# qasimyu/simuscop

Measured on AMD Instinct MI355X. Metric: simulated paired reads/sec (whole node) at 30x WGS PE150, higher is better.
Workload: dtype u32

## Files before the change

simuscop_amd/csrc/sg_emit_fast.hip:

```cpp
#include "sg_emit.h"

namespace sg {

__device__ __forceinline__ uint32_t pack4(uint32_t w) {
  return (w | (w >> 6) | (w >> 12) | (w >> 18)) & 0xFFu;
}

typedef uint32_t u32x2 __attribute__((ext_vector_type(2)));
typedef uint32_t u32x4 __attribute__((ext_vector_type(4)));

#define FAST_CTX 192u

#define BITOP_OR_AND 0xF8
#define BITOP_XOR_AND 0x78
#define BITOP_ANDN_OR 0xBA

__device__ __noinline__ uint32_t tail_word(uint32_t slot, uint32_t c, uint32_t h, uint32_t c3b, uint32_t k0, uint32_t k1) {
  uint32_t y[4];
  philox_base(slot, 2u * c + (h >> 2), 1u, c3b, k0, k1, y);
  const uint32_t l = h & 3u;
  return l == 0u ? y[0] : l == 1u ? y[1] : l == 2u ? y[2] : y[3];
}

template <int H>
__device__ __forceinline__ void sample1(uint32_t col_sh, uint32_t col_mask, uint32_t cw, uint32_t wh, uint32_t so_h, uint32_t qo_h, uint32_t cd4_w,
                                        uint32_t& acc, uint32_t& sy) {
  typedef const __attribute__((address_space(3))) uint32_t* lds_word;
  const uint32_t kv4 = (cw >> (2 * H + 4)) & 0xFCu;
  const uint32_t keepm1 = *(lds_word)(uintptr_t)(so_h + kv4);
  const uint32_t d_s = keepm1 - (wh >> 16);
  const uint32_t col16 = (wh >> col_sh) & col_mask;
  const uint32_t qa = qo_h + ((cd4_w >> (8 * (H & 3))) & 0xFFu);
  const uint32_t e = *(lds_word)(uintptr_t)(qa + col16 + FAST_CTX * 4u);
  const uint32_t d_q = (wh & 0xFFFFu) - (e & 0xFFFFu);
  const uint32_t z = __builtin_amdgcn_bitop3_b32(d_q - 1u, d_q, d_s, BITOP_ANDN_OR);
  acc = __builtin_amdgcn_bitop3_b32(acc, z, 1u << (17 + H), BITOP_OR_AND);
  sy = __builtin_amdgcn_bitop3_b32(e >> 8, e, d_q, BITOP_XOR_AND);
}

__device__ __forceinline__ void sample8(const uint32_t* code4, uint32_t lgW, uint32_t cw, const uint32_t (&x)[8],
                                        const uint32_t (&so)[8], uint32_t qo0, uint32_t qo1, uint32_t (&sw)[2], uint32_t (&qw)[2],
                                        uint32_t& acc_out) {
  const uint32_t cd4[2] = {code4[(cw >> 10) & 0xFFu], code4[(cw >> 18) & 0xFFu]};
  const uint32_t col_sh = 12u - lgW, col_mask = ((1u << lgW) - 1u) << 4;
  uint32_t acc = 0, sy[8];
  sample1<0>(col_sh, col_mask, cw, x[0], so[0], qo0, cd4[0], acc, sy[0]);
  sample1<1>(col_sh, col_mask, cw, x[1], so[1], qo1, cd4[0], acc, sy[1]);
  sample1<2>(col_sh, col_mask, cw, x[2], so[2], so[2], cd4[0], acc, sy[2]);
  sample1<3>(col_sh, col_mask, cw, x[3], so[3], so[3], cd4[0], acc, sy[3]);
  sample1<4>(col_sh, col_mask, cw, x[4], so[4], so[4], cd4[1], acc, sy[4]);
  sample1<5>(col_sh, col_mask, cw, x[5], so[5], so[5], cd4[1], acc, sy[5]);
  sample1<6>(col_sh, col_mask, cw, x[6], so[6], so[6], cd4[1], acc, sy[6]);
  sample1<7>(col_sh, col_mask, cw, x[7], so[7], so[7], cd4[1], acc, sy[7]);
#pragma unroll
  for (int g = 0; g < 2; g++) {
    const uint32_t p01 = __builtin_amdgcn_perm(sy[4 * g + 1], sy[4 * g], 0x0C0C0602u);
    const uint32_t p23 = __builtin_amdgcn_perm(sy[4 * g + 3], sy[4 * g + 2], 0x06020C0Cu);
    qw[g] = p01 | p23;
    sw[g] = __builtin_amdgcn_perm(0u, 0x47544341u, cd4[g] >> 2);
  }
  acc_out = acc;
}

__device__ __forceinline__ void store_var(uint8_t* q, uint64_t lo, uint64_t hi, uint32_t n) {
  if (n >= 8u) {
    __builtin_memcpy(q, &lo, 8);
    if (n > 8u) {
      const uint32_t k = 8u * (n - 8u);
      const uint64_t v = (lo >> k) | (hi << (64u - k));
      __builtin_memcpy(q + n - 8u, &v, 8);
    }
  } else if (n >= 4u) {
    const uint32_t a = (uint32_t)lo, b = (uint32_t)(lo >> (8u * (n - 4u)));
    __builtin_memcpy(q, &a, 4);
    if (n > 4u) __builtin_memcpy(q + n - 4u, &b, 4);
  } else if (n >= 2u) {
    const uint16_t a = (uint16_t)lo, b = (uint16_t)(lo >> (8u * (n - 2u)));
    __builtin_memcpy(q, &a, 2);
    if (n > 2u) __builtin_memcpy(q + n - 2u, &b, 2);
  } else if (n == 1u) {
    *q = (uint8_t)lo;
  }
}

constexpr uint32_t FAST_G = 63u;

template <bool PAIRED, bool DIAG>
struct FastBlock {
  const DevProfile& P;
  const DevBatch& B;
  uint32_t m, tm;
  uint32_t dg;
  uint32_t bins, TI, inv_TI, clean_cap;
  uint32_t img_at;
  const uint32_t* lut;
  const uint32_t* code4;
  bool tail_whole;
  uint32_t TIp;
  uint32_t TI16, inv_TI16;

  __device__ __forceinline__ FastBlock(const DevProfile& P_, const DevBatch& B_, uint32_t m_, uint32_t TI_, uint32_t inv_TI_,
                                       uint32_t clean_cap_, uint32_t img_at_, const uint32_t* lut_, const uint32_t* code4_)
      : P(P_), B(B_), m(m_), tm(PAIRED ? m_ : 0u), dg(DIAG ? B_.diag : 0u), bins((uint32_t)P_.bins), TI(TI_), inv_TI(inv_TI_),
        clean_cap(clean_cap_), img_at(img_at_), lut(lut_), code4(code4_) {
    tail_whole = ((uint32_t)P.L & 7u) == 7u && ((uint32_t)P.L + 7u) / 8u == TI;
    TIp = tail_whole ? TI : TI - 1u;
    TI16 = (tail_whole ? TIp - 1u : TIp) >> 1;
    inv_TI16 = TI16 ? (1u << 20) / TI16 + 1u : 0u;
  }
  __device__ __forceinline__ bool rc(bool row_bit) const { return PAIRED ? m == 1u : row_bit; }
  __device__ __forceinline__ uint2 fetch_window(bool row_bit, uint32_t idx) const {
    uint2 v;
    fetch_window(row_bit, idx, v);
    return v;
  }
  __device__ __forceinline__ void fetch_window(bool row_bit, uint32_t idx, uint2& into) const {
    __builtin_memcpy(&into, (rc(row_bit) ? B.chains2_rc : B.chains2_fwd) + (idx >> 2), 8);
  }
  __device__ __forceinline__ uint32_t c3b() const { return dev_ctx(KIND_BASE, m, B.batch_id); }
};

__device__ __forceinline__ uint64_t window_codes(uint2 w, uint32_t idx) { return (((uint64_t)w.y << 32) | w.x) >> (2u * (idx & 3u)); }

struct FastWave {
  uint32_t lane;
  FastRows rows;
  uint32_t* slow_list;
  uint2* fix_list;
  uint8_t* perm;
  uint8_t* permp;
  uint16_t* ovf;
  uint16_t* clean;
  uint32_t g;
  uint8_t* gout;
  __amdgpu_buffer_rsrc_t out_rsrc;
  uint32_t nslow, nfix;
  __device__ __forceinline__ unsigned long long lanes_below() const { return (1ull << lane) - 1ull; }
};

template <bool PAIRED, bool DIAG>
__device__ __forceinline__ void heads8(const FastBlock<PAIRED, DIAG>& k, uint32_t slot, uint32_t c, uint32_t (&x)[8]) {
  const uint32_t c3b = k.c3b();
  if (k.dg & 8u) {
#pragma unroll
    for (int z = 0; z < 8; z++) x[z] = (slot * 2654435761u) ^ (c * 40503u + z * 0x9E3779B9u);
  } else {
    philox_base(slot, 2u * c, 0, c3b, k.B.k0, k.B.k1, x);
    philox_base(slot, 2u * c + 1u, 0, c3b, k.B.k0, k.B.k1, x + 4);
  }
}

template <class S, class Fetch, class Run>
__device__ __forceinline__ void pipelined_steps(S cur, uint32_t first, uint32_t last, Fetch fetch, Run run) {
  for (uint32_t step = first; step < last; step++) {
    const S nxt = fetch(min(step + 1u, last - 1u));
    run(cur);
    cur = nxt;
  }
}

template <bool PAIRED, bool DIAG>
__device__ __forceinline__ void flush_slow(const FastBlock<PAIRED, DIAG>& k, FastWave& w) {
  const DevBatch& B = k.B;
  const uint32_t m = k.m, lane = w.lane;
  wave_lds_sync();
  uint32_t base = 0;
  if (lane == 0u) base = atomicAdd(B.slowq_count + m, w.nslow);
  base = (uint32_t)__builtin_amdgcn_readfirstlane((int)base);
  for (uint32_t b0 = 0; b0 < w.nslow; b0 += 64u) {
    const uint32_t i = b0 + lane;
    if (i < w.nslow && base + i < B.slowq_cap) {
      const uint32_t e = w.slow_list[i];
      B.slowq[(size_t)m * B.slowq_cap + base + i] = make_uint2(w.g * FAST_G + (e & 0xFFu), e >> 8);
    }
  }
  if (lane == 0u && base + w.nslow > B.slowq_cap) atomicOr((unsigned long long*)(B.totals + 3), 2ull);
  w.nslow = 0;
  wave_lds_sync();
}

template <bool PAIRED, bool DIAG>
__device__ __forceinline__ void flush_fix(const FastBlock<PAIRED, DIAG>& k, FastWave& w) {
  const DevProfile& P = k.P;
  const DevBatch& B = k.B;
  const uint32_t bins = k.bins, lane = w.lane;
  wave_lds_sync();
  __builtin_amdgcn_s_waitcnt(0x0F70);
  const uint32_t lgW = P.lgW, u_mask = (1u << (16u - lgW)) - 1u;
  const uint4* gsub = P.fast_sub + (size_t)k.tm * bins * FAST_CTX;
  const uint32_t c3b = k.c3b();
  for (uint32_t b0 = 0; b0 < w.nfix; b0 += 64u) {
    const uint2 fe = w.fix_list[b0 + lane < w.nfix ? b0 + lane : 0u];
    uint32_t todo = b0 + lane < w.nfix ? (fe.x >> 6) & 0xFFu : 0u;
    const uint32_t r = fe.x & 63u, c = fe.x >> 17, cw = fe.y;
    const uint32_t slot = w.g * FAST_G + r + B.slot_offset;
    const FastRow rr = w.rows.load(r);
    const uint32_t np = rr.np(), hl = rr.hdr_len();
    const bool whole = 8u * c + 8u <= np + (uint32_t)((np & 7u) == 7u);
    const uint32_t inv = row::inv_of(max(np, 1u));
    while (__ballot(todo != 0u) != 0ull) {
      const bool on = todo != 0u;
      const uint32_t h = on ? (uint32_t)__builtin_ctz(todo) : 0u;
      todo &= todo - 1u;
      const uint32_t i = 8u * c + h;
      const uint32_t bin = __umulhi(__umul24(i, bins), inv);
      uint32_t xw[4];
      philox_base(slot, 2u * c + (h >> 2), 0, c3b, B.k0, B.k1, xw);
      const uint32_t l = h & 3u;
      const uint32_t wh = l == 0u ? xw[0] : l == 1u ? xw[1] : l == 2u ? xw[2] : xw[3];
      const uint32_t region = c == 0u ? (h == 0u ? 128u : h == 1u ? 64u : 0u) : 0u;
      const uint32_t cdn = (cw >> (2u * h + 10u)) & 3u;
      const uint4 row = gsub[(size_t)bin * FAST_CTX + region + ((cw >> (2u * h + 6u)) & 63u)];
      const uint32_t sh = wh >> 16, h0 = row.x >> 16, h1 = row.y >> 16, h2 = row.z >> 16;
      const uint32_t jj = (uint32_t)(sh > h0) + (uint32_t)(sh > h1) + (uint32_t)(sh > h2);
      const bool amb_s = on && jj != (uint32_t)(sh >= h0) + (uint32_t)(sh >= h1) + (uint32_t)(sh >= h2);
      uint32_t kn = 0;
      uint2 e2 = make_uint2(0, 0);
      const uint32_t col = (wh & 0xFFFFu) >> (16u - lgW), uh = wh & u_mask;
      auto column = [&](uint32_t j_) {
        const uint32_t jm = max(j_, row.w & 3u);
        kn = (row.w >> (2u * jm + 2u)) & 3u;
        e2 = P.fast_alias[((((size_t)cdn * 4u + kn) * bins + bin) << lgW) + col];
      };
      if (!amb_s) column(jj);
      const bool need_tail = amb_s || (on && uh == (e2.x >> 16) && (e2.y & 0xFFu) != (e2.y >> 8));
      uint32_t wt = 0;
      if (__ballot(need_tail) != 0ull) {
        if (need_tail) wt = tail_word(slot, c, h, c3b, B.k0, B.k1);
      }
      if (__ballot(amb_s) != 0ull) {
        if (amb_s) {
          const uint32_t xs = (wh & 0xFFFF0000u) | (wt >> 16);
          column((uint32_t)(xs > row.x) + (uint32_t)(xs > row.y) + (uint32_t)(xs > row.z));
        }
      }
      const uint32_t th = e2.x >> 16;
      const bool lo_side = uh != th ? uh < th : ((uh << 16) | (wt & 0xFFFFu)) < e2.x;
      const uint32_t sym = (lo_side ? (e2.y & 0xFFu) : (e2.y >> 8)) + (uint32_t)P.min_qual;
      const uint32_t ch = (0x47544341u >> (8u * kn)) & 0xFFu;
      if (on) {
        if (whole) {
          uint8_t* rec = w.gout + rr.out_off() + hl + i;
          rec[0] = (uint8_t)ch;
          rec[np + 3u] = (uint8_t)sym;
        } else if (!rr.parked_slow()) {
          w.rows.patch_parked(r, h, ch, sym);
        }
      }
    }
  }
  w.nfix = 0;
  wave_lds_sync();
}

template <bool PAIRED, bool DIAG>
__device__ __forceinline__ void push_fix(const FastBlock<PAIRED, DIAG>& k, FastWave& w, uint32_t r, uint32_t c, uint32_t fix, uint32_t cw) {
  const unsigned long long fm = __ballot(fix != 0u);
  if (fm) {
    if (w.nfix + 64u > FIX_CAP) flush_fix(k, w);
    if (fix != 0u) w.fix_list[w.nfix + (uint32_t)__popcll(fm & w.lanes_below())] = make_uint2(r | (fix << 6) | (c << 17), cw);
    w.nfix += (uint32_t)__popcll(fm);
  }
}

__device__ __forceinline__ void stage_tables(const DevProfile& P, uint32_t tm, uint32_t TI, uint32_t* img, uint32_t img_at,
                                             uint32_t* lut, uint32_t* code4) {
  const uint32_t tid = threadIdx.x, bins = (uint32_t)P.bins, img_words = bins * P.fast_stride;
  const uint4* src = (const uint4*)(P.fast_lds + (size_t)tm * P.fast_mate_words);
  for (uint32_t i = tid; i < (img_words + 3u) / 4u; i += EMIT_THREADS) ((uint4*)img)[i] = src[i];
  const uint32_t blk_bytes = P.fast_stride * 4u;
  for (uint32_t i = tid; i < TI * LUT_ROW; i += EMIT_THREADS) {
    const uint32_t c = i / LUT_ROW, f = i - c * LUT_ROW;
    const uint32_t h = f < 8u ? f : f - 8u;
    const uint32_t pos = 8u * c + h;
    const uint32_t bin = min(pos * bins / (uint32_t)P.L, bins - 1u);
    uint32_t v = bin * blk_bytes;
    if (f < 8u && c == 0u) v += f == 0u ? 128u * 4u : f == 1u ? 64u * 4u : 0u;
    lut[i] = f < 10u ? v + img_at : 0u;
  }
  for (uint32_t i = tid; i < 256u; i += EMIT_THREADS) {
    uint32_t v = 0;
    for (uint32_t z = 0; z < 4u; z++) v |= (((i >> (2u * z)) & 3u) * 4u) << (8u * z);
    code4[i] = v;
  }
}

template <bool PAIRED>
__device__ __forceinline__ void store_name(const DevBatch& B, uint32_t m, const ReadRow& my, size_t idx, uint8_t* rec) {
  const uint32_t nv = my.hdr_len() - B.prefix_len;
  if (__builtin_expect(nv > 16u, 0)) {
    write_name(rec, B.prefix, B.prefix_len, my.namepos(), my.fragcount(), PAIRED ? 1u : 0u, m);
    return;
  }
  const uint64_t p_lo = ((uint64_t)B.prefix_w[1] << 32) | B.prefix_w[0], p_hi = ((uint64_t)B.prefix_w[3] << 32) | B.prefix_w[2];
  const uint4 tx = B.meta[idx * 3 + 2];
  const uint64_t b0 = ((uint64_t)tx.y << 32) | tx.x, b1 = ((uint64_t)tx.w << 32) | tx.z;
  const uint32_t plen = B.prefix_len, hb = plen + nv;
  if (plen < 16u && hb >= 16u && hb <= 24u) {
    const uint32_t sh = 8u * plen;
    uint64_t w0, w1, w2;
    if (sh < 64u) {
      w0 = p_lo | (b0 << sh);
      w1 = p_hi | (b1 << sh) | (sh ? b0 >> (64u - sh) : 0ull);
      w2 = sh ? b1 >> (64u - sh) : 0ull;
    } else {
      const uint32_t t2 = sh - 64u;
      w0 = p_lo;
      w1 = p_hi | (b0 << t2);
      w2 = (b1 << t2) | (t2 ? b0 >> (64u - t2) : 0ull);
    }
    struct { uint64_t a, b; } first = {w0, w1};
    __builtin_memcpy(rec, &first, 16);
    const uint32_t n2 = hb - 16u;
    if (n2) {
      const uint32_t k = 8u * n2;
      const uint64_t v = k == 64u ? w2 : (w1 >> k) | (w2 << (64u - k));
      __builtin_memcpy(rec + hb - 8u, &v, 8);
    }
  } else {
    if (plen == 16u) { __builtin_memcpy(rec, &p_lo, 8); __builtin_memcpy(rec + 8, &p_hi, 8); }
    else store_var(rec, p_lo, p_hi, plen);
    uint8_t* q = rec + plen;
    if (nv == 16u) __builtin_memcpy(q, &tx, 16);
    else store_var(q, b0, b1, nv);
  }
}

__device__ __forceinline__ uint64_t open_group(FastWave& w, uint8_t* out, uint64_t ooff) {
  const uint64_t gbase = ((uint64_t)(uint32_t)__builtin_amdgcn_readfirstlane((int)(ooff >> 32)) << 32) |
                         (uint32_t)__builtin_amdgcn_readfirstlane((int)(uint32_t)ooff);
  w.gout = out + gbase;
  w.out_rsrc = __builtin_amdgcn_make_buffer_rsrc(w.gout, 0, 0x80000000u, 0x00020000);
  return gbase;
}

struct GroupPlan {
  uint32_t items;
  bool plain_l, split_l;
  bool small;
  uint32_t extra;
  uint32_t kb, ca0, n_whole, ka, n_gen, vscan;
  unsigned long long m_plain, m_rest, m_one, m_multi, b1, b2;
  uint32_t n_plain, n_psingle, n_rest, n_one, n_fast, n_single, n_gen_all, n_moved;
  uint32_t n_clean, n_ovf;
  unsigned long long more;
};

template <bool PAIRED, bool DIAG>
__device__ __forceinline__ void split_one_indel_reads(const FastBlock<PAIRED, DIAG>& k, const FastWave& w, const ReadRow& my, GroupPlan& gp) {
  const uint32_t TI = k.TI, lane = w.lane, items = gp.items, np_l = my.np();
  const bool act_l = items > 0u, plain_l = gp.plain_l;
  gp.kb = 0; gp.ca0 = 0; gp.n_whole = 0; gp.ka = 0; gp.n_gen = 0; gp.vscan = 0;
  gp.split_l = false;
  const bool cand0_l = act_l && my.nev() == 1u && !my.bad_block();
  if (k.clean_cap != 0u && (uint32_t)__popcll(__ballot(cand0_l)) * (TI - 2u) >= 96u) {
    const uint32_t ew = my.event();
    const uint32_t ej = ew & 0xFFFFu, elen = (ew >> 16) & 0x7FFFu;
    const bool del = (ew >> 31) != 0u;
    const uint32_t fc = del ? ej : ej + 1u, fs = del ? ej : ej + elen + 1u;
    gp.n_whole = np_l >> 3;
    gp.kb = min(fc >> 3, gp.n_whole);
    gp.ca0 = (fs + 12u) >> 3;
    gp.ka = gp.n_whole > gp.ca0 ? gp.n_whole - gp.ca0 : 0u;
    gp.n_gen = gp.ka ? (gp.ca0 - gp.kb) + (items - gp.n_whole) : items - gp.kb;
    const bool cand_l = cand0_l && items <= 255u && gp.kb + gp.ka != 0u;
    uint32_t v = cand_l ? ((gp.kb + gp.ka) << 16) | gp.n_gen : 0u;
#pragma unroll
    for (int d = 1; d < 64; d <<= 1) {
      const uint32_t up = __shfl_up(v, d, 64);
      if ((int)lane >= d) v += up;
    }
    gp.vscan = v;
    const uint32_t extra_l = items > TI ? items - TI : 0u;
    const uint32_t others = (k.tail_whole ? 0u : (uint32_t)__popcll(__ballot(plain_l))) +
                            (uint32_t)__popcll(__ballot(extra_l == 1u || extra_l == 2u)) + (uint32_t)__popcll(__ballot(extra_l == 2u));
    bool split_l = cand_l && (v >> 16) <= k.clean_cap && others + (v & 0xFFFFu) <= OVF_CAP;
    const unsigned long long ms = __ballot(split_l);
    if (ms) {
      const uint32_t tot_s = (uint32_t)__shfl((int)v, 63 - __builtin_clzll(ms), 64);
      const uint32_t n_cl = tot_s >> 16, n_gn = tot_s & 0xFFFFu;
      const uint32_t whole = (uint32_t)__popcll(__ballot(act_l && !plain_l && !split_l));
      const uint32_t s0 = (whole + (uint32_t)__popcll(ms)) * TI + others, s1 = whole * TI + others + n_gn;
      const uint32_t rem = n_cl & 63u, mv = (rem != 0u && rem <= ((0u - s1) & 63u)) ? rem : 0u;
      const uint32_t before = 48u * ((s0 + 63u) >> 6);
      const uint32_t after = 26u * ((n_cl - mv + 63u) >> 6) + 48u * ((s1 + mv + 63u) >> 6) + 25u;
      if (after >= before) split_l = false;
    }
    gp.split_l = split_l;
    gp.kb = split_l ? gp.kb : 0u;
    gp.ka = split_l ? gp.ka : 0u;
    gp.n_gen = split_l ? gp.n_gen : 0u;
  }
}

template <bool PAIRED, bool DIAG>
__device__ __forceinline__ GroupPlan classify_group(const FastBlock<PAIRED, DIAG>& k, const FastWave& w, const ReadRow& my, uint32_t items) {
  GroupPlan gp;
  const uint32_t TI = k.TI;
  const uint32_t nev_l = my.nev();
  const bool act_l = items > 0u;
  gp.items = items;
  gp.plain_l = act_l && nev_l == 0u && my.np() == (uint32_t)k.P.L && items == TI && !my.bad_block() && k.TIp != 0u;
  split_one_indel_reads(k, w, my, gp);
  const bool plain_l = gp.plain_l, split_l = gp.split_l;
  const unsigned long long m_split = __ballot(split_l);
  gp.m_plain = __ballot(plain_l);
  gp.m_multi = __ballot(act_l && nev_l >= 2u);
  gp.m_one = __ballot(act_l && nev_l == 1u && !split_l);
  gp.m_rest = __ballot(act_l && !plain_l && nev_l == 0u);
  gp.n_plain = (uint32_t)__popcll(gp.m_plain);
  gp.n_psingle = k.tail_whole ? 0u : gp.n_plain;
  gp.n_rest = (uint32_t)__popcll(gp.m_rest);
  gp.n_one = (uint32_t)__popcll(gp.m_one);
  gp.n_fast = gp.n_rest + gp.n_one + (uint32_t)__popcll(gp.m_multi);
  gp.extra = (items > TI && !split_l) ? items - TI : 0u;
  gp.small = gp.extra == 1u || gp.extra == 2u;
  gp.b1 = __ballot(gp.small);
  gp.b2 = __ballot(gp.extra == 2u);
  gp.n_single = gp.n_psingle + (uint32_t)__popcll(gp.b1) + (uint32_t)__popcll(gp.b2);
  const uint32_t tot = m_split ? (uint32_t)__shfl((int)gp.vscan, 63 - __builtin_clzll(m_split), 64) : 0u;
  gp.n_clean = tot >> 16;
  gp.n_gen_all = tot & 0xFFFFu;
  gp.n_moved = 0;
  {
    const uint32_t rem = gp.n_clean & 63u, idle = (0u - (gp.n_fast * TI + gp.n_single + gp.n_gen_all)) & 63u;
    if (rem != 0u && rem <= idle && gp.n_single + gp.n_gen_all + rem <= OVF_CAP) gp.n_moved = rem;
  }
  gp.n_ovf = gp.n_moved + gp.n_single + gp.n_gen_all;
  gp.more = (k.dg & 256u) ? 0ull : __ballot(gp.extra > 2u);
  return gp;
}

template <bool PAIRED, bool DIAG>
__device__ __forceinline__ void compose_lists(const FastBlock<PAIRED, DIAG>& k, const FastWave& w, GroupPlan& gp) {
  const uint32_t TI = k.TI, lane = w.lane, items = gp.items, n_moved = gp.n_moved;
  const unsigned long long lt = w.lanes_below();
  if (items > 0u && !gp.split_l) {
    if (gp.plain_l) {
      const uint32_t pos = (uint32_t)__popcll(gp.m_plain & lt);
      w.permp[pos] = (uint8_t)lane;
      if (!k.tail_whole) w.ovf[n_moved + pos] = (uint16_t)(lane | (k.TIp << 8));
    } else {
      uint32_t pos;
      if ((gp.m_rest >> lane) & 1ull) pos = (uint32_t)__popcll(gp.m_rest & lt);
      else if ((gp.m_one >> lane) & 1ull) pos = gp.n_rest + (uint32_t)__popcll(gp.m_one & lt);
      else pos = gp.n_rest + gp.n_one + (uint32_t)__popcll(gp.m_multi & lt);
      w.perm[pos] = (uint8_t)lane;
    }
  }
  if (gp.n_fast == 0u && lane == 0u) w.perm[0] = 0;
  if (gp.small) {
    const uint32_t o = n_moved + gp.n_psingle + (uint32_t)__popcll(gp.b1 & lt) + (uint32_t)__popcll(gp.b2 & lt);
    w.ovf[o] = (uint16_t)(lane | (TI << 8));
    if (gp.extra == 2u) w.ovf[o + 1u] = (uint16_t)(lane | ((TI + 1u) << 8));
  }
  if (gp.split_l) {
    const uint32_t kb = gp.kb, ka = gp.ka, ca0 = gp.ca0;
    const uint32_t oc = (gp.vscan >> 16) - (kb + ka);
    uint32_t og = n_moved + gp.n_single + (gp.vscan & 0xFFFFu) - gp.n_gen;
    const uint32_t kt = kb + ka, behind = ((ca0 - kb) << 7) | 64u;
    for (uint32_t q = 0; q < kt; q++) w.clean[oc + q] = (uint16_t)((lane | (q << 7)) + (q >= kb ? behind : 0u));
    const uint32_t mid_end = ka ? ca0 : items;
    for (uint32_t c = kb; c < mid_end; c++) w.ovf[og++] = (uint16_t)(lane | (c << 8));
    if (ka) for (uint32_t c = gp.n_whole; c < items; c++) w.ovf[og++] = (uint16_t)(lane | (c << 8));
  }
  wave_lds_sync();
  if (n_moved) {
    gp.n_clean -= n_moved;
    if (lane < n_moved) {
      const uint32_t e = w.clean[gp.n_clean + lane];
      w.ovf[lane] = (uint16_t)((e & 63u) | ((e >> 7) << 8));
    }
    wave_lds_sync();
  }
}

struct PlainSteps {
  bool use16;
  uint32_t n_plain, np16steps, cnt8, c8_base, n_pitems, npsteps;
};
template <bool PAIRED, bool DIAG>
__device__ __forceinline__ PlainSteps plan_plain_steps(const FastBlock<PAIRED, DIAG>& k, uint32_t n_plain) {
  PlainSteps ps;
  const uint32_t dg = k.dg, TIp = k.TIp, TI16 = k.TI16;
  ps.n_plain = n_plain;
  ps.use16 = !(dg & 512u) && TIp >= 18u;
  const uint32_t n_p16 = ps.use16 ? n_plain * TI16 : 0u;
  ps.np16steps = (dg & 128u) ? 0u : n_p16 >> 6;
  const uint32_t rem16 = n_p16 - (ps.np16steps << 6);
  ps.cnt8 = ps.use16 ? TIp - 2u * TI16 : TIp;
  ps.c8_base = ps.use16 ? 2u * TI16 : 0u;
  ps.n_pitems = 2u * rem16 + n_plain * ps.cnt8;
  ps.npsteps = (dg & 128u) ? 0u : (ps.n_pitems + 63u) / 64u;
  return ps;
}

__device__ __forceinline__ void lut_bins(const uint32_t* lut, uint32_t c, uint32_t (&so)[8], uint32_t& qo0, uint32_t& qo1) {
  const uint4* lrow = (const uint4*)(lut + c * LUT_ROW);
  const uint4 r0 = lrow[0], r1 = lrow[1], r2 = lrow[2];
  so[0] = r0.x; so[1] = r0.y; so[2] = r0.z; so[3] = r0.w; so[4] = r1.x; so[5] = r1.y; so[6] = r1.z; so[7] = r1.w;
  qo0 = r2.x; qo1 = r2.y;
}

struct P16 { uint32_t r, c, src, out; uint2 w; };

template <bool PAIRED, bool DIAG>
__device__ __forceinline__ void plain16_step(const FastBlock<PAIRED, DIAG>& k, FastWave& w, const P16& st, uint32_t qual_at) {
  const uint32_t dg = k.dg;
  const uint32_t c8 = 2u * st.c;
  const uint64_t w64 = window_codes(st.w, st.src);
  uint32_t cwa = (uint32_t)w64, cwb = (uint32_t)(w64 >> 16);
  const uint32_t slot = w.g * FAST_G + st.r + k.B.slot_offset;
  if (dg & 4u) { cwa = (w.g * FAST_G + st.r) * 2654435761u + c8; cwb = cwa * 40503u + 1u; }
  uint32_t sw[4], qw[4], fixv[2];
#pragma unroll
  for (int hf = 0; hf < 2; hf++) {
    uint32_t x[8];
    const uint32_t c = c8 + (uint32_t)hf, cw = hf ? cwb : cwa;
    heads8(k, slot, c, x);
    uint32_t so[8], qo0, qo1;
    lut_bins(k.lut, c, so, qo0, qo1);
    uint32_t s2[2], q2[2], acc;
    sample8(k.code4, k.P.lgW, cw, x, so, qo0, qo1, s2, q2, acc);
    sw[2 * hf] = s2[0]; sw[2 * hf + 1] = s2[1];
    qw[2 * hf] = q2[0]; qw[2 * hf + 1] = q2[1];
    fixv[hf] = (dg & 16u) ? 0u : (acc >> 17) & 0xFFu;
  }
  const uint32_t so_ = (dg & 1u) ? 0xFFFFFFFFu : st.out;
  const uint32_t qo_ = (dg & 1u) ? 0xFFFFFFFFu : st.out + qual_at;
  __builtin_amdgcn_raw_buffer_store_b128(u32x4{sw[0], sw[1], sw[2], sw[3]}, w.out_rsrc, so_, 0, 0);
  __builtin_amdgcn_raw_buffer_store_b128(u32x4{qw[0], qw[1], qw[2], qw[3]}, w.out_rsrc, qo_, 0, 0);
#pragma unroll
  for (int hf = 0; hf < 2; hf++) push_fix(k, w, st.r, c8 + (uint32_t)hf, fixv[hf], hf ? cwb : cwa);
}

template <bool PAIRED, bool DIAG>
__device__ __forceinline__ void plain16_steps(const FastBlock<PAIRED, DIAG>& k, FastWave& w, uint32_t a16, uint32_t b16) {
  uint32_t TI16_v = k.TI16, inv_TI16_v = k.inv_TI16, qual_at = (uint32_t)k.P.L + 3u;
  asm volatile("" : "+v"(TI16_v), "+v"(inv_TI16_v), "+v"(qual_at));
  auto fetch16 = [&](uint32_t step) -> P16 {
    P16 st;
    const uint32_t i = step * 64u + w.lane;
    const uint32_t ri = __umul24(i, inv_TI16_v) >> 20;
    st.c = i - __umul24(ri, TI16_v);
    st.r = w.permp[ri];
    const uint32_t A = w.rows.src_word(st.r);
    st.src = row::src_m5(A) + 16u * st.c;
    st.out = w.rows.base_off(st.r) + 16u * st.c;
    st.w = k.fetch_window(row::copy_is_rc(A), st.src);
    return st;
  };
  P16 cur = fetch16(a16);
  __builtin_amdgcn_raw_buffer_store_b128(u32x4{0u, 0u, 0u, 0u}, w.out_rsrc, 0xFFFFFFFFu, 0, 0);
  __builtin_amdgcn_raw_buffer_store_b128(u32x4{0u, 0u, 0u, 0u}, w.out_rsrc, 0xFFFFFFF0u, 0, 0);
  pipelined_steps(cur, a16, b16, fetch16, [&](const P16& st) { plain16_step(k, w, st, qual_at); });
}

template <bool PAIRED, bool DIAG>
__device__ __forceinline__ void sample_store8(const FastBlock<PAIRED, DIAG>& k, FastWave& w, uint32_t r, uint32_t c, bool ok, uint2 win,
                                              uint32_t src, const uint32_t (&so)[8], uint32_t qo0, uint32_t qo1, uint32_t out,
                                              uint32_t qual_at, bool tail_patch) {
  const uint32_t dg = k.dg;
  uint32_t cw;
  if (dg & 4u) cw = (w.g * FAST_G + r) * 2654435761u + c;
  else cw = (uint32_t)window_codes(win, src);
  uint32_t x[8];
  heads8(k, w.g * FAST_G + r + k.B.slot_offset, c, x);
  uint32_t sw[2], qw[2], acc;
  sample8(k.code4, k.P.lgW, cw, x, so, qo0, qo1, sw, qw, acc);
  const bool st_ok = ok && !(dg & 1u);
  const uint32_t so_ = st_ok ? out : 0xFFFFFFFFu;
  const uint32_t qo_ = st_ok ? out + qual_at : 0xFFFFFFFFu;
  uint32_t fix_mask = 0xFFu;
  if (tail_patch) {
    const bool last = c + 1u == k.TI;
    const uint32_t sel = last ? 0x04020100u : 0x03020100u;
    sw[1] = __builtin_amdgcn_perm(0x0Au, sw[1], sel);
    qw[1] = __builtin_amdgcn_perm(0x0Au, qw[1], sel);
    __builtin_amdgcn_raw_buffer_store_b16((unsigned short)0x0A2Bu, w.out_rsrc, st_ok && last ? so_ + 8u : 0xFFFFFFFFu, 0, 0);
    fix_mask = last ? 0x7Fu : 0xFFu;
  }
  __builtin_amdgcn_raw_buffer_store_b64(u32x2{sw[0], sw[1]}, w.out_rsrc, so_, 0, 0);
  __builtin_amdgcn_raw_buffer_store_b64(u32x2{qw[0], qw[1]}, w.out_rsrc, qo_, 0, 0);
  const uint32_t fix = (ok && !(dg & 16u)) ? (acc >> 17) & fix_mask : 0u;
  push_fix(k, w, r, c, fix, cw);
}

struct PStage { uint32_t r, c, src, out; bool ok; uint2 w; };

template <bool PAIRED, bool DIAG>
__device__ __forceinline__ void plain8_steps(const FastBlock<PAIRED, DIAG>& k, FastWave& w, const PlainSteps& ps, uint32_t a8, uint32_t b8) {
  const uint32_t cnt8 = ps.cnt8, c8_base = ps.c8_base, n_pitems = ps.n_pitems, TI16 = k.TI16, inv_TI16 = k.inv_TI16;
  uint32_t qual_at = (uint32_t)k.P.L + 3u, n_single = ps.n_plain * cnt8, i16_base = ps.np16steps << 6;
  asm volatile("" : "+v"(qual_at), "+v"(n_single), "+v"(i16_base));
  const uint32_t inv_cnt8 = cnt8 ? (1u << 20) / cnt8 + 1u : 0u;
  auto fetch_plain = [&](uint32_t step) -> PStage {
    PStage st;
    const uint32_t i_raw = step * 64u + w.lane;
    st.ok = i_raw < n_pitems;
    const uint32_t i = min(i_raw, n_pitems - 1u);
    const bool half = i >= n_single;
    const uint32_t j = i - n_single;
    const uint32_t q = half ? i16_base + (j >> 1) : i;
    const uint32_t d = half ? TI16 : cnt8;
    const uint32_t ri = __umul24(q, half ? inv_TI16 : inv_cnt8) >> 20;
    const uint32_t rem = q - __umul24(ri, d);
    st.c = half ? 2u * rem + (j & 1u) : c8_base + rem;
    st.r = w.permp[ri];
    const uint32_t A = w.rows.src_word(st.r);
    st.src = row::src_m5(A) + 8u * st.c;
    st.out = w.rows.base_off(st.r) + 8u * st.c;
    st.w = k.fetch_window(row::copy_is_rc(A), st.src);
    return st;
  };
  auto run_plain = [&](const PStage& st) {
    uint32_t so[8], qo0, qo1;
    lut_bins(k.lut, st.c, so, qo0, qo1);
    sample_store8(k, w, st.r, st.c, st.ok, st.w, st.src, so, qo0, qo1, st.out, qual_at, k.tail_whole);
  };
  PStage cur = fetch_plain(a8);
  __builtin_amdgcn_raw_buffer_store_b64(u32x2{0u, 0u}, w.out_rsrc, 0xFFFFFFFFu, 0, 0);
  __builtin_amdgcn_raw_buffer_store_b64(u32x2{0u, 0u}, w.out_rsrc, 0xFFFFFFF0u, 0, 0);
  if (k.tail_whole) __builtin_amdgcn_raw_buffer_store_b16((unsigned short)0u, w.out_rsrc, 0xFFFFFFE0u, 0, 0);
  pipelined_steps(cur, a8, b8, fetch_plain, run_plain);
}

template <bool PAIRED, bool DIAG>
__device__ __forceinline__ void plain_steps(const FastBlock<PAIRED, DIAG>& k, FastWave& w, uint32_t n_plain) {
  const PlainSteps ps = plan_plain_steps(k, n_plain);
  const uint32_t h16 = ps.np16steps >> 1, s8_first = (ps.use16 && ps.cnt8 && ps.npsteps) ? 1u : 0u;
#pragma unroll 1
  for (uint32_t ph = 0; ph < 2u; ph++) {
    const uint32_t a16 = ph ? h16 : 0u, b16 = ph ? ps.np16steps : h16;
    const uint32_t a8 = ph ? s8_first : 0u, b8 = ph ? ps.npsteps : s8_first;
    if (a16 < b16) plain16_steps(k, w, a16, b16);
    if (a8 < b8) plain8_steps(k, w, ps, a8, b8);
  }
}

struct CStage { uint32_t r, c, src, out, np, inv; bool ok; uint2 w; };

template <bool PAIRED, bool DIAG>
__device__ __forceinline__ void clean_steps(const FastBlock<PAIRED, DIAG>& k, FastWave& w, uint32_t n_clean) {
  if (!n_clean) return;
  const uint32_t ncsteps = (k.dg & 128u) ? 0u : (n_clean + 63u) / 64u;
  auto fetch_clean = [&](uint32_t step) -> CStage {
    CStage st;
    const uint32_t i_raw = step * 64u + w.lane;
    st.ok = i_raw < n_clean;
    const uint32_t e = w.clean[min(i_raw, n_clean - 1u)];
    st.r = e & 63u;
    st.c = e >> 7;
    const FastRow q = w.rows.load(st.r);
    const uint32_t elen = (q.event() >> 16) & 0x7FFFu;
    const uint32_t delta = (e & 64u) ? ((q.event() >> 31) ? elen : 0u - elen) : 0u;
    st.src = q.src_m5() + 8u * st.c + delta;
    st.out = q.base_off() + 8u * st.c;
    st.np = q.np();
    st.inv = q.inv();
    st.w = k.fetch_window(q.copy_is_rc(), st.src);
    return st;
  };
  const uint32_t bins = k.bins, blk_bytes = k.P.fast_stride * 4u;
  auto run_clean = [&](const CStage& st) {
    uint32_t so[8];
    const uint32_t ib0 = __umul24(8u * st.c, bins);
#pragma unroll
    for (int h = 0; h < 8; h++) so[h] = __umul24(__umulhi(ib0 + (uint32_t)h * bins, st.inv), blk_bytes) + k.img_at;
    const uint32_t qo0 = so[0], qo1 = so[1];
    if (st.c == 0u) { so[0] += 128u * 4u; so[1] += 64u * 4u; }
    sample_store8(k, w, st.r, st.c, st.ok, st.w, st.src, so, qo0, qo1, st.out, st.np + 3u, false);
  };
  if (ncsteps) {
    CStage cur = fetch_clean(0);
    __builtin_amdgcn_raw_buffer_store_b64(u32x2{0u, 0u}, w.out_rsrc, 0xFFFFFFFFu, 0, 0);
    __builtin_amdgcn_raw_buffer_store_b64(u32x2{0u, 0u}, w.out_rsrc, 0xFFFFFFF0u, 0, 0);
    pipelined_steps(cur, 0u, ncsteps, fetch_clean, run_clean);
  }
}

struct Stage { uint32_t r, c; bool active; FastRow row; uint32_t src; uint2 w; };

template <bool PAIRED, bool DIAG>
__device__ __forceinline__ uint32_t fast_src(const FastBlock<PAIRED, DIAG>& k, const FastRow& row, uint32_t c, bool active) {
  const uint32_t a = k.rc(row.rev()) ? (uint32_t)k.B.chains_total - row.frag_lo() - row.flen() : row.frag_lo();
  return active ? a + 8u * c - 5u : 128u;
}

template <bool PAIRED, bool DIAG>
__device__ __forceinline__ Stage fetch_item(const FastBlock<PAIRED, DIAG>& k, const FastWave& w, uint32_t r, uint32_t c, bool ok, uint32_t c_idle) {
  Stage st;
  st.r = r;
  st.row = w.rows.load(r);
  st.active = ok && st.row.active() && c < st.row.items();
  st.c = st.active ? c : c_idle;
  st.src = fast_src(k, st.row, st.c, st.active);
  st.w = k.fetch_window(st.row.rev(), st.src);
  return st;
}

template <bool PAIRED, bool DIAG>
__device__ __forceinline__ Stage fetch_step(const FastBlock<PAIRED, DIAG>& k, const FastWave& w, uint32_t n_items, uint32_t n_stream, uint32_t step) {
  const uint32_t i = step * 64u + w.lane;
  const bool ok = i < n_stream, in_map = i < n_items;
  const uint32_t ri = __umul24(i, k.inv_TI) >> 20;
  const uint32_t e = w.ovf[(ok && !in_map) ? i - n_items : 0u];
  const uint32_t r = in_map ? w.perm[ri] : (ok ? (e & 0xFFu) : w.perm[0]);
  const uint32_t c = in_map ? i - __umul24(ri, k.TI) : (ok ? e >> 8 : 1u);
  return fetch_item(k, w, r, c, ok, c);
}

struct ItemEvents { int d0; uint32_t n_in, ew_in, tj_in; };

template <bool PAIRED, bool DIAG>
__device__ __forceinline__ ItemEvents item_events(const FastBlock<PAIRED, DIAG>& k, const FastWave& w, const Stage& st) {
  const uint32_t nev_r = st.active ? st.row.nev() : 0u;
  const uint32_t c = st.c;
  ItemEvents ie;
  ie.d0 = 0;
  ie.n_in = nev_r == 1u ? 1u : 0u;
  ie.ew_in = st.row.event();
  ie.tj_in = st.row.event() & 0xFFFFu;
  if (__ballot(nev_r >= 2u) != 0ull) {
    if (nev_r >= 2u) {
      const uint32_t* ev = k.B.events + ((size_t)k.m * k.B.n_slots + (w.g * FAST_G + st.r)) * SG_MAX_EVENTS;
      const int p_lo = (int)(8u * c) - 2, p_hi = (int)(8u * c) + 7;
      int shift = 0;
      ie.n_in = 0;
      for (uint32_t q = 0; q < nev_r; q++) {
        const uint32_t e = ev[q];
        const int j = (int)(e & 0xFFFFu), len = (int)((e >> 16) & 0x7FFFu);
        const bool del = (e >> 31) != 0;
        const int pe = j + shift;
        if (del ? pe <= p_lo : pe + len < p_lo) { shift += del ? -len : len; continue; }
        if (del ? pe > p_hi : pe >= p_hi) break;
        if (ie.n_in == 0u) { ie.d0 = -shift; ie.ew_in = (e & 0xFFFF0000u) | (uint32_t)pe; ie.tj_in = (uint32_t)j; }
        ie.n_in++;
        shift += del ? -len : len;
      }
      if (ie.n_in == 0u) ie.d0 = -shift;
    }
  }
  return ie;
}

template <bool PAIRED, bool DIAG>
__device__ __forceinline__ uint32_t item_codes(const FastBlock<PAIRED, DIAG>& k, const Stage& st, uint2 wpre, const ItemEvents& ie, uint32_t nev, uint32_t slot) {
  const uint32_t c = st.c, i0 = 8u * c;
  const bool row_rev = st.row.rev();
  const uint32_t src = st.src + (uint32_t)ie.d0;
  if (__ballot(ie.d0 != 0) != 0ull) {
    if (ie.d0 != 0) k.fetch_window(row_rev, src, wpre);
  }
  uint32_t cw;
  if (k.dg & 4u) cw = slot * 2654435761u + c;
  else cw = (uint32_t)window_codes(wpre, src);

  if (__ballot(nev == 1u) != 0ull) {
    int q_ins = 1, q_end = 0;
    if (nev == 1u) {
      const uint32_t ew = ie.ew_in;
      const int ej = (int)(ew & 0xFFFFu), elen = (int)((ew >> 16) & 0x7FFFu);
      const bool del = (ew >> 31) != 0;
      const int delta = del ? elen : -elen;
      const uint32_t src2 = src + (uint32_t)delta;
      const uint32_t cw2 = (uint32_t)window_codes(k.fetch_window(row_rev, src2), src2);
      const int first_shifted = del ? ej : ej + elen + 1;
      const int q0 = first_shifted - ((int)i0 - 5);
      const uint32_t keep = q0 <= 0 ? 0u : (q0 >= 13 ? 0xFFFFFFFFu : ((1u << (2 * q0)) - 1u));
      cw = (cw & keep) | (cw2 & ~keep);
      if (!del) {
        q_ins = max(3, ej + 1 - ((int)i0 - 5));
        q_end = min(12, ej + elen - ((int)i0 - 5));
      }
    }
#pragma unroll 1
    for (; __ballot(q_ins <= q_end) != 0ull; q_ins++) {
      if (q_ins <= q_end) {
        const int p = (int)i0 - 5 + q_ins, ej = (int)(ie.ew_in & 0xFFFFu);
        const uint32_t prof = __umulhi(aux_draw(k.B, slot, ie.tj_in, (uint32_t)(p - ej), k.m), 3u);
        const uint32_t nat = (k.P.inv_remap_packed >> (2u * prof)) & 3u;
        cw = (cw & ~(3u << (2 * q_ins))) | (nat << (2 * q_ins));
      }
    }
  }
  return cw;
}

template <bool PAIRED, bool DIAG>
__device__ __forceinline__ void item_bins(const FastBlock<PAIRED, DIAG>& k, const Stage& st, uint32_t (&so)[8], uint32_t& qo0, uint32_t& qo1) {
  const uint32_t c = st.c, bins = k.bins, blk_bytes = k.P.fast_stride * 4u;
  const bool active = st.active;
  const bool lut_ok = st.row.np() == (uint32_t)k.P.L && c < k.TI;
  if (__ballot(active && !lut_ok) == 0ull) {
    lut_bins(k.lut, lut_ok ? c : 0u, so, qo0, qo1);
  } else {
    const uint32_t ib0 = __umul24(8u * c, bins), inv = st.row.inv();
#pragma unroll
    for (int h = 0; h < 8; h++) {
      const uint32_t bin = __umulhi(ib0 + (uint32_t)h * bins, inv);
      so[h] = __umul24(active ? bin : 0u, blk_bytes) + k.img_at;
    }
    qo0 = so[0]; qo1 = so[1];
    if (c == 0u) { so[0] += 128u * 4u; so[1] += 64u * 4u; }
  }
}

template <bool PAIRED, bool DIAG>
__device__ __forceinline__ void store_item(const FastBlock<PAIRED, DIAG>& k, const FastWave& w, const Stage& st, bool slow,
                                           const uint32_t (&sw)[2], const uint32_t (&qw)[2]) {
  const uint32_t np = st.row.np(), i0 = 8u * st.c;
  const bool active = st.active, go = active && !slow;
  const bool last7 = i0 + 7u == np;
  const bool whole = i0 + 8u <= np || last7;
  const bool sto = go && whole && !(k.dg & 1u);
  const uint32_t so_ = sto ? st.row.out_off() + st.row.hdr_len() + i0 : 0xFFFFFFFFu;
  const uint32_t qo_ = sto ? so_ + np + 3u : 0xFFFFFFFFu;
  const uint32_t s1 = last7 ? (sw[1] & 0x00FFFFFFu) | 0x0A000000u : sw[1];
  const uint32_t q1 = last7 ? (qw[1] & 0x00FFFFFFu) | 0x0A000000u : qw[1];
  __builtin_amdgcn_raw_buffer_store_b64(u32x2{sw[0], s1}, w.out_rsrc, so_, 0, 0);
  __builtin_amdgcn_raw_buffer_store_b64(u32x2{qw[0], q1}, w.out_rsrc, qo_, 0, 0);
  __builtin_amdgcn_raw_buffer_store_b16((unsigned short)0x0A2Bu, w.out_rsrc, sto && last7 ? so_ + 8u : 0xFFFFFFFFu, 0, 0);
  if (active && i0 + 8u > np && !(last7 && !slow)) w.rows.park(st.r, slow, sw, qw);
}

template <bool PAIRED, bool DIAG>
__device__ __forceinline__ bool fast_item(const FastBlock<PAIRED, DIAG>& k, const FastWave& w, const Stage& st, const ItemEvents& ie,
                                          uint32_t& fix, uint32_t& cw_out) {
  const bool active = st.active;
  const uint32_t c = st.c, slot = w.g * FAST_G + st.r;
  const uint32_t np = st.row.np(), nev = active ? ie.n_in : 0u;
  const uint32_t bad = st.row.bad_block();
  const uint32_t cw = item_codes(k, st, st.w, ie, nev, slot);
  uint32_t x[8];
  heads8(k, slot + k.B.slot_offset, c, x);
  uint32_t so[8], qo0, qo1;
  item_bins(k, st, so, qo0, qo1);
  uint32_t qw[2], sw[2], acc;
  sample8(k.code4, k.P.lgW, cw, x, so, qo0, qo1, sw, qw, acc);
  const bool slow = active && (bad != 0u || nev >= 2u);
  fix = (active && !slow && !(k.dg & 16u)) ? (acc >> 17) & 0xFFu & ((1u << min(8u, np - 8u * c)) - 1u) : 0u;
  cw_out = cw;
  store_item(k, w, st, slow, sw, qw);
  return slow;
}

template <bool PAIRED, bool DIAG>
__device__ __forceinline__ void general_step(const FastBlock<PAIRED, DIAG>& k, FastWave& w, const Stage& st) {
  const ItemEvents ie = item_events(k, w, st);
  uint32_t fix, cw;
  const bool slow = fast_item(k, w, st, ie, fix, cw);
  const unsigned long long sm = __ballot(slow);
  if (sm) {
    if (slow) w.slow_list[w.nslow + (uint32_t)__popcll(sm & w.lanes_below())] = st.r | (st.c << 8);
    w.nslow += (uint32_t)__popcll(sm);
  }
  push_fix(k, w, st.r, st.c, fix, cw);
}

template <bool PAIRED, bool DIAG>
__device__ __forceinline__ void general_steps(const FastBlock<PAIRED, DIAG>& k, FastWave& w, const GroupPlan& gp) {
  const uint32_t n_items = gp.n_fast * k.TI, n_stream = n_items + gp.n_ovf;
  const uint32_t nmain = (k.dg & 256u) ? 0u : (n_stream + 63u) / 64u;
  if (!nmain) return;
  Stage cur = fetch_step(k, w, n_items, n_stream, 0u);
  __builtin_amdgcn_raw_buffer_store_b64(u32x2{0u, 0u}, w.out_rsrc, 0xFFFFFFFFu, 0, 0);
  __builtin_amdgcn_raw_buffer_store_b64(u32x2{0u, 0u}, w.out_rsrc, 0xFFFFFFF0u, 0, 0);
  __builtin_amdgcn_raw_buffer_store_b16((unsigned short)0u, w.out_rsrc, 0xFFFFFFE0u, 0, 0);
  pipelined_steps(
      cur, 0u, nmain,
      [&](uint32_t step) {
        if (w.nslow > SLOW_CAP - 64u) flush_slow(k, w);
// ... 137 lines not shown
```

Measured before the change: 2.145 billion.

## Stage sampling into phases with sched barriers to overlap LDS loads with Philox

Splits the per-8-base sampler into separate stages (code lookup, LDS address/keep loads, column LDS loads, decide, pack). Sched barriers interleave the two halves of each 16-base step so LDS latency is hidden behind the Philox head generation. The permuted read index for the next step is also prefetched one step ahead in the fetch lambda. This adds scheduling constraints that may raise register pressure and lower occupancy.

Result: no change. 2.159 billion (median of 6 runs) (+0.7%).

```diff
diff --git a/simuscop_amd/csrc/sg_emit_fast.hip b/simuscop_amd/csrc/sg_emit_fast.hip
--- a/simuscop_amd/csrc/sg_emit_fast.hip
+++ b/simuscop_amd/csrc/sg_emit_fast.hip
@@ -22,44 +22,79 @@
   return l == 0u ? y[0] : l == 1u ? y[1] : l == 2u ? y[2] : y[3];
 }
 
-template <int H>
-__device__ __forceinline__ void sample1(uint32_t col_sh, uint32_t col_mask, uint32_t cw, uint32_t wh, uint32_t so_h, uint32_t qo_h, uint32_t cd4_w,
-                                        uint32_t& acc, uint32_t& sy) {
-  typedef const __attribute__((address_space(3))) uint32_t* lds_word;
-  const uint32_t kv4 = (cw >> (2 * H + 4)) & 0xFCu;
-  const uint32_t keepm1 = *(lds_word)(uintptr_t)(so_h + kv4);
-  const uint32_t d_s = keepm1 - (wh >> 16);
-  const uint32_t col16 = (wh >> col_sh) & col_mask;
-  const uint32_t qa = qo_h + ((cd4_w >> (8 * (H & 3))) & 0xFFu);
-  const uint32_t e = *(lds_word)(uintptr_t)(qa + col16 + FAST_CTX * 4u);
-  const uint32_t d_q = (wh & 0xFFFFu) - (e & 0xFFFFu);
-  const uint32_t z = __builtin_amdgcn_bitop3_b32(d_q - 1u, d_q, d_s, BITOP_ANDN_OR);
-  acc = __builtin_amdgcn_bitop3_b32(acc, z, 1u << (17 + H), BITOP_OR_AND);
-  sy = __builtin_amdgcn_bitop3_b32(e >> 8, e, d_q, BITOP_XOR_AND);
+__device__ __forceinline__ void stage_fence() { __builtin_amdgcn_sched_barrier(0); }
+
+struct Block8 {
+  uint32_t cd4[2];
+  uint32_t k[8];
+  uint32_t q[8];
+};
+
+typedef const __attribute__((address_space(3))) uint32_t* lds_word;
+
+__device__ __forceinline__ void block8_codes(const uint32_t* code4, uint32_t cw, Block8& b) {
+  b.cd4[0] = code4[(cw >> 10) & 0xFFu];
+  b.cd4[1] = code4[(cw >> 18) & 0xFFu];
+}
+
+template <int H0, int N>
+__device__ __forceinline__ void block8_addr(uint32_t cw, const uint32_t (&so)[8], uint32_t qo0, uint32_t qo1, Block8& b) {
+#pragma unroll
+  for (int h = H0; h < H0 + N; h++) {
+    const uint32_t kv4 = (cw >> (2 * h + 4)) & 0xFCu;
+    b.k[h] = *(lds_word)(uintptr_t)(so[h] + kv4);
+    const uint32_t qo_h = h == 0 ? qo0 : h == 1 ? qo1 : so[h];
+    b.q[h] = qo_h + ((b.cd4[h >> 2] >> (8 * (h & 3))) & 0xFFu);
+  }
+}
+
+template <int H0, int N>
+__device__ __forceinline__ void block8_cols(uint32_t lgW, const uint32_t (&x)[8], Block8& b) {
+  const uint32_t col_sh = 12u - lgW, col_mask = ((1u << lgW) - 1u) << 4;
+#pragma unroll
+  for (int h = H0; h < H0 + N; h++) {
+    const uint32_t col16 = (x[h] >> col_sh) & col_mask;
+    b.q[h] = *(lds_word)(uintptr_t)(b.q[h] + col16 + FAST_CTX * 4u);
+  }
+}
+
+template <int H0, int N>
+__device__ __forceinline__ void block8_decide(const uint32_t (&x)[8], const Block8& b, uint32_t& acc, uint32_t (&sy)[8]) {
+#pragma unroll
+  for (int h = H0; h < H0 + N; h++) {
+    const uint32_t wh = x[h], e = b.q[h];
+    const uint32_t d_s = b.k[h] - (wh >> 16);
+    const uint32_t d_q = (wh & 0xFFFFu) - (e & 0xFFFFu);
+    const uint32_t z = __builtin_amdgcn_bitop3_b32(d_q - 1u, d_q, d_s, BITOP_ANDN_OR);
+    acc = __builtin_amdgcn_bitop3_b32(acc, z, 1u << (17 + h), BITOP_OR_AND);
+    sy[h] = __builtin_amdgcn_bitop3_b32(e >> 8, e, d_q, BITOP_XOR_AND);
+  }
+}
+
+template <int G>
+__device__ __forceinline__ void block8_pack(const Block8& b, const uint32_t (&sy)[8], uint32_t (&sw)[2], uint32_t (&qw)[2]) {
+  const uint32_t p01 = __builtin_amdgcn_perm(sy[4 * G + 1], sy[4 * G], 0x0C0C0602u);
+  const uint32_t p23 = __builtin_amdgcn_perm(sy[4 * G + 3], sy[4 * G + 2], 0x06020C0Cu);
+  qw[G] = p01 | p23;
+  sw[G] = __builtin_amdgcn_perm(0u, 0x47544341u, b.cd4[G] >> 2);
+}
+
+__device__ __forceinline__ void block8_finish(const uint32_t (&x)[8], const Block8& b, uint32_t (&sw)[2], uint32_t (&qw)[2], uint32_t& acc_out) {
+  uint32_t acc = 0, sy[8];
+  block8_decide<0, 8>(x, b, acc, sy);
+  block8_pack<0>(b, sy, sw, qw);
+  block8_pack<1>(b, sy, sw, qw);
+  acc_out = acc;
 }
 
 __device__ __forceinline__ void sample8(const uint32_t* code4, uint32_t lgW, uint32_t cw, const uint32_t (&x)[8],
                                         const uint32_t (&so)[8], uint32_t qo0, uint32_t qo1, uint32_t (&sw)[2], uint32_t (&qw)[2],
                                         uint32_t& acc_out) {
-  const uint32_t cd4[2] = {code4[(cw >> 10) & 0xFFu], code4[(cw >> 18) & 0xFFu]};
-  const uint32_t col_sh = 12u - lgW, col_mask = ((1u << lgW) - 1u) << 4;
-  uint32_t acc = 0, sy[8];
-  sample1<0>(col_sh, col_mask, cw, x[0], so[0], qo0, cd4[0], acc, sy[0]);
-  sample1<1>(col_sh, col_mask, cw, x[1], so[1], qo1, cd4[0], acc, sy[1]);
-  sample1<2>(col_sh, col_mask, cw, x[2], so[2], so[2], cd4[0], acc, sy[2]);
-  sample1<3>(col_sh, col_mask, cw, x[3], so[3], so[3], cd4[0], acc, sy[3]);
-  sample1<4>(col_sh, col_mask, cw, x[4], so[4], so[4], cd4[1], acc, sy[4]);
-  sample1<5>(col_sh, col_mask, cw, x[5], so[5], so[5], cd4[1], acc, sy[5]);
-  sample1<6>(col_sh, col_mask, cw, x[6], so[6], so[6], cd4[1], acc, sy[6]);
-  sample1<7>(col_sh, col_mask, cw, x[7], so[7], so[7], cd4[1], acc, sy[7]);
-#pragma unroll
-  for (int g = 0; g < 2; g++) {
-    const uint32_t p01 = __builtin_amdgcn_perm(sy[4 * g + 1], sy[4 * g], 0x0C0C0602u);
-    const uint32_t p23 = __builtin_amdgcn_perm(sy[4 * g + 3], sy[4 * g + 2], 0x06020C0Cu);
-    qw[g] = p01 | p23;
-    sw[g] = __builtin_amdgcn_perm(0u, 0x47544341u, cd4[g] >> 2);
-  }
-  acc_out = acc;
+  Block8 b;
+  block8_codes(code4, cw, b);
+  block8_addr<0, 8>(cw, so, qo0, qo1, b);
+  block8_cols<0, 8>(lgW, x, b);
+  block8_finish(x, b, sw, qw, acc_out);
 }
 
 __device__ __forceinline__ void store_var(uint8_t* q, uint64_t lo, uint64_t hi, uint32_t n) {
@@ -138,16 +173,19 @@
   __device__ __forceinline__ unsigned long long lanes_below() const { return (1ull << lane) - 1ull; }
 };
 
-template <bool PAIRED, bool DIAG>
-__device__ __forceinline__ void heads8(const FastBlock<PAIRED, DIAG>& k, uint32_t slot, uint32_t c, uint32_t (&x)[8]) {
-  const uint32_t c3b = k.c3b();
+template <int J, bool PAIRED, bool DIAG>
+__device__ __forceinline__ void heads4(const FastBlock<PAIRED, DIAG>& k, uint32_t slot, uint32_t c, uint32_t (&x)[8]) {
   if (k.dg & 8u) {
 #pragma unroll
-    for (int z = 0; z < 8; z++) x[z] = (slot * 2654435761u) ^ (c * 40503u + z * 0x9E3779B9u);
+    for (int z = 4 * J; z < 4 * J + 4; z++) x[z] = (slot * 2654435761u) ^ (c * 40503u + z * 0x9E3779B9u);
   } else {
-    philox_base(slot, 2u * c, 0, c3b, k.B.k0, k.B.k1, x);
-    philox_base(slot, 2u * c + 1u, 0, c3b, k.B.k0, k.B.k1, x + 4);
-  }
+    philox_base(slot, 2u * c + (uint32_t)J, 0, k.c3b(), k.B.k0, k.B.k1, x + 4 * J);
+  }
+}
+template <bool PAIRED, bool DIAG>
+__device__ __forceinline__ void heads8(const FastBlock<PAIRED, DIAG>& k, uint32_t slot, uint32_t c, uint32_t (&x)[8]) {
+  heads4<0>(k, slot, c, x);
+  heads4<1>(k, slot, c, x);
 }
 
 template <class S, class Fetch, class Run>
@@ -512,20 +550,32 @@
   uint32_t cwa = (uint32_t)w64, cwb = (uint32_t)(w64 >> 16);
   const uint32_t slot = w.g * FAST_G + st.r + k.B.slot_offset;
   if (dg & 4u) { cwa = (w.g * FAST_G + st.r) * 2654435761u + c8; cwb = cwa * 40503u + 1u; }
-  uint32_t sw[4], qw[4], fixv[2];
-#pragma unroll
-  for (int hf = 0; hf < 2; hf++) {
-    uint32_t x[8];
-    const uint32_t c = c8 + (uint32_t)hf, cw = hf ? cwb : cwa;
-    heads8(k, slot, c, x);
-    uint32_t so[8], qo0, qo1;
-    lut_bins(k.lut, c, so, qo0, qo1);
-    uint32_t s2[2], q2[2], acc;
-    sample8(k.code4, k.P.lgW, cw, x, so, qo0, qo1, s2, q2, acc);
-    sw[2 * hf] = s2[0]; sw[2 * hf + 1] = s2[1];
-    qw[2 * hf] = q2[0]; qw[2 * hf + 1] = q2[1];
-    fixv[hf] = (dg & 16u) ? 0u : (acc >> 17) & 0xFFu;
-  }
+  uint32_t soA[8], qoA0, qoA1, soB[8], qoB0, qoB1, xa[8], xb[8];
+  Block8 a, b;
+  lut_bins(k.lut, c8, soA, qoA0, qoA1);
+  block8_codes(k.code4, cwa, a);
+  lut_bins(k.lut, c8 + 1u, soB, qoB0, qoB1);
+  block8_codes(k.code4, cwb, b);
+  stage_fence();
+  block8_addr<0, 8>(cwa, soA, qoA0, qoA1, a);
+  stage_fence();
+  heads8(k, slot, c8, xa);
+  stage_fence();
+  block8_cols<0, 8>(k.P.lgW, xa, a);
+  block8_addr<0, 8>(cwb, soB, qoB0, qoB1, b);
+  stage_fence();
+  heads8(k, slot, c8 + 1u, xb);
+  stage_fence();
+  block8_cols<0, 8>(k.P.lgW, xb, b);
+  stage_fence();
+  uint32_t sw[4], qw[4], fixv[2], s2[2], q2[2], acc;
+  block8_finish(xa, a, s2, q2, acc);
+  sw[0] = s2[0]; sw[1] = s2[1]; qw[0] = q2[0]; qw[1] = q2[1];
+  fixv[0] = (dg & 16u) ? 0u : (acc >> 17) & 0xFFu;
+  stage_fence();
+  block8_finish(xb, b, s2, q2, acc);
+  sw[2] = s2[0]; sw[3] = s2[1]; qw[2] = q2[0]; qw[3] = q2[1];
+  fixv[1] = (dg & 16u) ? 0u : (acc >> 17) & 0xFFu;
   const uint32_t so_ = (dg & 1u) ? 0xFFFFFFFFu : st.out;
   const uint32_t qo_ = (dg & 1u) ? 0xFFFFFFFFu : st.out + qual_at;
   __builtin_amdgcn_raw_buffer_store_b128(u32x4{sw[0], sw[1], sw[2], sw[3]}, w.out_rsrc, so_, 0, 0);
@@ -538,16 +588,19 @@
 __device__ __forceinline__ void plain16_steps(const FastBlock<PAIRED, DIAG>& k, FastWave& w, uint32_t a16, uint32_t b16) {
   uint32_t TI16_v = k.TI16, inv_TI16_v = k.inv_TI16, qual_at = (uint32_t)k.P.L + 3u;
   asm volatile("" : "+v"(TI16_v), "+v"(inv_TI16_v), "+v"(qual_at));
+  auto read_of = [&](uint32_t step) { return (uint32_t)w.permp[__umul24(step * 64u + w.lane, inv_TI16_v) >> 20]; };
+  uint32_t r_nxt = read_of(a16);
   auto fetch16 = [&](uint32_t step) -> P16 {
     P16 st;
     const uint32_t i = step * 64u + w.lane;
     const uint32_t ri = __umul24(i, inv_TI16_v) >> 20;
     st.c = i - __umul24(ri, TI16_v);
-    st.r = w.permp[ri];
+    st.r = r_nxt;
     const uint32_t A = w.rows.src_word(st.r);
     st.src = row::src_m5(A) + 16u * st.c;
     st.out = w.rows.base_off(st.r) + 16u * st.c;
     st.w = k.fetch_window(row::copy_is_rc(A), st.src);
+    r_nxt = read_of(min(step + 1u, b16 - 1u));
     return st;
   };
   P16 cur = fetch16(a16);
@@ -564,10 +617,26 @@
   uint32_t cw;
   if (dg & 4u) cw = (w.g * FAST_G + r) * 2654435761u + c;
   else cw = (uint32_t)window_codes(win, src);
-  uint32_t x[8];
-  heads8(k, w.g * FAST_G + r + k.B.slot_offset, c, x);
-  uint32_t sw[2], qw[2], acc;
-  sample8(k.code4, k.P.lgW, cw, x, so, qo0, qo1, sw, qw, acc);
+  const uint32_t slot = w.g * FAST_G + r + k.B.slot_offset, lgW = k.P.lgW;
+  uint32_t x[8], sw[2], qw[2], sy[8], acc = 0;
+  Block8 b;
+  block8_codes(k.code4, cw, b);
+  stage_fence();
+  block8_addr<0, 8>(cw, so, qo0, qo1, b);
+  stage_fence();
+  heads4<0>(k, slot, c, x);
+  stage_fence();
+  block8_cols<0, 4>(lgW, x, b);
+  stage_fence();
+  heads4<1>(k, slot, c, x);
+  stage_fence();
+  block8_cols<4, 4>(lgW, x, b);
+  stage_fence();
+  block8_decide<0, 4>(x, b, acc, sy);
+  block8_pack<0>(b, sy, sw, qw);
+  stage_fence();
+  block8_decide<4, 4>(x, b, acc, sy);
+  block8_pack<1>(b, sy, sw, qw);
   const bool st_ok = ok && !(dg & 1u);
   const uint32_t so_ = st_ok ? out : 0xFFFFFFFFu;
   const uint32_t qo_ = st_ok ? out + qual_at : 0xFFFFFFFFu;
```
